# taraak/pita

Hardware: AMD Instinct MI355X
Metric: walker-steps/sec (batch x T) LJ13 @ 65k walkers/GPU (higher is better)
Workload: dtype f32

## Files before the change

pita_amd/csrc/egnn_div_kernel.hip:

```cpp
#include <type_traits>

#include "egnn_common.h"

namespace pita {

struct DivParams {
  const unsigned* mats16;
  const unsigned* mats16h;
  const float* vecs;
  const float* vecs_h;
  const float* vecs_div;
  float* cache;
  int* mark;
  int repair;
  int nchunk;
  int* bad_flag;
  int bad_seq;
  int n_layers, in_nf, attention, tanh_on, feature_layout;
  float coord_scale;
  long long B;
  const float* h;
  const float* x;
  const float* beta;
  int dir0, ndir;
  long long cache_waves;
  float* diag_acc;
  float* out;
  int no_mean;
  const float* probes;
  unsigned long long seed, walker_offset;
  long long step;
  float* q_out;
};

template <int N, int DIM>
__device__ __forceinline__ void probe_values(const DivParams& p, int probe, long long wid, int node, float (&v)[DIM]) {
  if (p.probes) {
    const float* src = p.probes + (((long long)probe * p.B + wid) * N + node) * DIM;
#pragma unroll
    for (int k = 0; k < DIM; ++k) v[k] = src[k];
  } else {
    const uint32_t word = philox_rademacher_word(p.seed, p.walker_offset + (unsigned long long)wid, p.step, (uint32_t)probe,
                                                 (uint32_t)node);
#pragma unroll
    for (int k = 0; k < DIM; ++k) v[k] = rademacher_sign(word, k);
  }
}

template <int N, int DIM, int POS_F>
__device__ __forceinline__ float probe_quadratic_form(const float* dscr, const float* vtab, int w, int d, float c_s, float cf) {
  const float* dF = dscr + d * POS_F + w * N * DIM;
  const float* vv = vtab + d * POS_F + w * N * DIM;
  float mean[DIM];
#pragma unroll
  for (int c = 0; c < DIM; ++c) {
    float s = 0.f;
    for (int j = 0; j < N; ++j) s += dF[j * DIM + c];
    mean[c] = s / (float)N;
  }
  float q = 0.f;
  for (int i = 0; i < N; ++i)
#pragma unroll
    for (int c = 0; c < DIM; ++c) {
      const float v = vv[i * DIM + c];
      q = fmaf(v, fmaf(cf, dF[i * DIM + c] - mean[c], c_s * v), q);
    }
  return q;
}

template <int N, int DIM, int G, int WAVES, int K, int DAL = 1>
struct DivCfg {
  static constexpr int NCOL = G * N;
  static constexpr int NT = (NCOL + 31) / 32;
  static constexpr int NCOLP = NT * 32;
  static constexpr int PB_F = NCOLP * PBS;
  static constexpr int POS_F = NCOLP * DIM;
  static constexpr int WAVE_F = (1 + K + DAL * K) * PB_F + 3 * POS_F + 3 * K * POS_F;
  static __host__ __device__ constexpr int vec_f(int L) { return ((VEC_EMB_F + L * VEC_LAYER_F) + 3) & ~3; }
  static __host__ __device__ constexpr size_t lds_bytes(int L) {
    return sizeof(float) * (size_t)(vec_f(L) + WAVES * WAVE_F + L * VEC_DIV_F);
  }
// ... 288 lines not shown
        }
      }
      wave_lds_fence();
      cur ^= 1;
    }

    float* dscr = dPB;
#pragma unroll
    for (int T = 0; T < NT; ++T)
#pragma unroll
      for (int d = 0; d < K; ++d)
#pragma unroll
        for (int k = 0; k < DIM; ++k) {
          dposi[T][d][k] -= dp0i[T][d][k];
          if (hh == 0) dscr[d * C::POS_F + col[T] * DIM + k] = dposi[T][d][k];
        }
    if constexpr (PROBE) {
      float* vtab = dA;
#pragma unroll
      for (int T = 0; T < NT; ++T) {
        const long long wid = valid[T] ? walker0 + col[T] / N : p.B - 1;
#pragma unroll
        for (int d = 0; d < K; ++d) {
          float pv[DIM];
          probe_values<N, DIM>(p, dir0 + (d < ndir ? d : 0), wid, nodei[T], pv);
          if (hh == 0) {
#pragma unroll
            for (int k = 0; k < DIM; ++k) vtab[d * C::POS_F + col[T] * DIM + k] = (valid[T] && d < ndir) ? pv[k] : 0.f;
          }
        }
      }
      wave_lds_fence();
      if (lane < G * K) {
        const int w = lane / K, d = lane - w * K;
        if (w < nwalk && d < ndir && (!p.repair || p.mark[walker0 + w] != 0)) {
          const float hv = p.h[walker0 + w];
          const float op = 1.0f + hv, rs = 1.0f / sqrtf(op);
          p.q_out[(long long)(dir0 + d) * p.B + walker0 + w] =
              probe_quadratic_form<N, DIM, C::POS_F>(dscr, vtab, w, d, 1.0f / op, sqrtf(hv) * rs);
        }
      }
      wave_lds_fence();
    } else {
    wave_lds_fence();
#pragma unroll
    for (int T = 0; T < NT; ++T) {
      const int cb = (col[T] < ncol) ? col[T] - nodei[T] : 0;
#pragma unroll
      for (int d = 0; d < K; ++d)
#pragma unroll
        for (int k = 0; k < DIM; ++k) {
          if (!(mine[T] && hh == 0 && d < ndir && nodei[T] * DIM + k == dir0 + d)) continue;
          float ds = 0.f;
          for (int q = 0; q < N; ++q) ds += dscr[d * C::POS_F + (cb + q) * DIM + k];
          const float dF = p.no_mean ? dposi[T][d][k] : dposi[T][d][k] - ds / (float)N;
          atomicAdd(&p.diag_acc[walker0 + col[T] / N], fmaf(c_out[T], dF, c_s[T]));
        }
    }
    wave_lds_fence();
    }
    if (p.out && ch == 0) {
      float* scr = PB;
#pragma unroll
      for (int T = 0; T < NT; ++T)
        if (hh == 0) {
#pragma unroll
          for (int k = 0; k < DIM; ++k) scr[col[T] * DIM + k] = posi[T][k] - p0i[T][k];
        }
      wave_lds_fence();
#pragma unroll
      for (int T = 0; T < NT; ++T) {
        if (!(mine[T] && hh == 0)) continue;
        const int cb = col[T] - nodei[T];
#pragma unroll
        for (int k = 0; k < DIM; ++k) {
          float sum = 0.f;
          for (int q = 0; q < N; ++q) sum += scr[(cb + q) * DIM + k];
          const float F = (posi[T][k] - p0i[T][k]) - sum / (float)N;
          const long long gi = (walker0 * N + col[T]) * DIM + k;
          p.out[gi] = fmaf(c_s[T], p.x[gi], c_out[T] * F);
        }
      }
      wave_lds_fence();
    }
    }
  }
}


template <int N, int DIM, int NT>
struct DivCache {
  static constexpr int POSX = NT * 32 * DIM;
  static constexpr int POSF = ((POSX + 2 * NT * 32 + 255) / 256) * 256;
  static __host__ __device__ int nvec(int l, int L) { return (l == 0 || l == L - 1) ? 1 : 4; }
  static __host__ __device__ size_t edge_f(int l, int L) { return (size_t)nvec(l, L) * 1024 + 512; }
  static __host__ __device__ size_t gn_off(int l, int L) { return (size_t)(N - 1) * edge_f(l, L); }
  static __host__ __device__ size_t tile_f(int l, int L) { return 1024 + (size_t)(N - 1) * edge_f(l, L); }
  static __host__ __device__ size_t layer_f(int l, int L) { return POSF + (size_t)NT * tile_f(l, L); }
  static __host__ __device__ size_t group_f(int L) {
    size_t t = 0;
    for (int l = 0; l < L; ++l) t += layer_f(l, L);
    return t;
  }
  static __host__ __device__ size_t layer_off(int l, int L) {
    size_t t = 0;
    for (int q = 0; q < l; ++q) t += layer_f(q, L);
    return t;
  }
// ... 408 lines not shown
          gn *= F16_UNSCALE;
          if (clay) cache_store16(clay + CA::POSF + (size_t)T * CA::tile_f(l, L) + CA::gn_off(l, L), lane, gn);
          wn.load(nullptr, mats16h, M_WN2, lane);
          f32x16 o = wn.mul(yn, lds_vec16(vl + V_BN2 * EH));
          o *= F16_UNSCALE;
          hf[T] += o;
#pragma unroll
          for (int d = 0; d < K; ++d) {
            dzn[d] *= gn;
            f32x16 dho = wn.mul(dzn[d], zero16);
            dho *= F16_UNSCALE;
            dhf[T][d] += dho;
          }
        }
      }
      wave_lds_fence();
      cur ^= 1;
    }

    float* dscr = dPB;
    float* tsl = PB;
#pragma unroll
    for (int T = 0; T < NT; ++T)
#pragma unroll
      for (int d = 0; d < K; ++d)
#pragma unroll
        for (int k = 0; k < DIM; ++k) {
          dposi[T][d][k] -= dp0i[T][d][k];
          if (hh == 0) dscr[d * C::POS_F + col[T] * DIM + k] = dposi[T][d][k];
        }
    if (lane < G * K) tsl[lane] = 0.f;
    if constexpr (PROBE) {
      const float* vtab = dpos0;
      wave_lds_fence();
      if (lane < G * K) {
        const int w = lane / KA, d = lane - w * KA;
        if (w < nwalk && d < p.ndir) {
          const float hv = p.h[walker0 + w];
          const float op = 1.0f + hv, rs = 1.0f / sqrtf(op);
          tsl[lane] = probe_quadratic_form<N, DIM, C::POS_F>(dscr, vtab, w, d, 1.0f / op, (sqrtf(hv) * rs) * rs);
        }
      }
    } else {
    wave_lds_fence();
#pragma unroll
    for (int T = 0; T < NT; ++T) {
      const int cb = (col[T] < ncol) ? col[T] - nodei[T] : 0;
#pragma unroll
      for (int d = 0; d < K; ++d)
#pragma unroll
        for (int k = 0; k < DIM; ++k) {
          if (!(valid[T] && hh == 0 && d < p.ndir && nodei[T] * DIM + k == p.dir0 + d)) continue;
          float ds = 0.f;
          for (int q = 0; q < N; ++q) ds += dscr[d * C::POS_F + (cb + q) * DIM + k];
          const float dF = p.no_mean ? dposi[T][d][k] : dposi[T][d][k] - ds / (float)N;
          tsl[(col[T] / N) * K + d] = fmaf(c_out[T] * c_in[T], dF, c_s[T]);
        }
    }
    }
    wave_lds_fence();
    bool bad[NT];
#pragma unroll
    for (int T = 0; T < NT; ++T) {
      bad[T] = false;
      if constexpr (K > 0) {
        const int w = col[T] / N;
        float sum = 0.f;
#pragma unroll
        for (int d = 0; d < K; ++d) sum += tsl[(valid[T] ? w : 0) * K + d];
        bad[T] = valid[T] && !__builtin_isfinite(sum);
        if (valid[T] && hh == 0 && nodei[T] == 0) {
          if constexpr (PROBE) {
            if (!bad[T])
#pragma unroll
              for (int d = 0; d < K; ++d)
                if (d < p.ndir) p.q_out[(long long)(p.dir0 + d) * p.B + walker0 + w] = tsl[w * K + d];
          } else {
            if (!bad[T]) p.diag_acc[walker0 + w] += sum;
          }
          p.mark[walker0 + w] = bad[T] ? 1 : 0;
          if (bad[T] && p.bad_flag) *p.bad_flag = p.bad_seq;
        }
      }
    }
    wave_lds_fence();
    if (p.out || K == 0) {
      float* scr = PB;
#pragma unroll
      for (int T = 0; T < NT; ++T)
        if (hh == 0) {
#pragma unroll
          for (int k = 0; k < DIM; ++k) scr[col[T] * DIM + k] = posi[T][k] - p0i[T][k];
        }
      wave_lds_fence();
#pragma unroll
      for (int T = 0; T < NT; ++T) {
        if (!(valid[T] && hh == 0) || bad[T]) continue;
        const int cb = col[T] - nodei[T];
        float F[DIM];
        bool fin = true;
#pragma unroll
        for (int k = 0; k < DIM; ++k) {
          float sum = 0.f;
          for (int q = 0; q < N; ++q) sum += scr[(cb + q) * DIM + k];
          F[k] = (posi[T][k] - p0i[T][k]) - sum / (float)N;
          fin = fin && __builtin_isfinite(F[k]);
        }
        if constexpr (K == 0) {
// ... 248 lines not shown
            if (hh == 0) dposb[(2 * d + (cur ^ 1)) * C::POS_F + col[T] * DIM + k] = dposi[T][d][k];
          }
        if (l != L - 1) {
          const f32x16 gn = cache_load16(ctile + CA::gn_off(l, L), lane);
          WFrag<2> wn;
          f32x16 dzn[K];
          if (!first) {
            wn.load(nullptr, mats16h, M_WN1A, lane);
#pragma unroll
            for (int d = 0; d < K; ++d) dzn[d] = wn.mul(dhf[T][d], zero16);
          } else {
#pragma unroll
            for (int d = 0; d < K; ++d) dzn[d] = zero16;
          }
          wn.load(nullptr, mats16h, M_WN1B, lane);
#pragma unroll
          for (int d = 0; d < K; ++d) dzn[d] = wn.mul(dagg[d], dzn[d]);
          wn.load(nullptr, mats16h, M_WN2, lane);
#pragma unroll
          for (int d = 0; d < K; ++d) {
            dzn[d] *= gn;
            f32x16 dho = wn.mul(dzn[d], zero16);
            dho *= F16_UNSCALE;
            dhf[T][d] += dho;
          }
        }
      }
      wave_lds_fence();
      cur ^= 1;
    }

    float* dscr = dPB;
    float* tsl = dPB + K * C::POS_F;
#pragma unroll
    for (int T = 0; T < NT; ++T)
#pragma unroll
      for (int d = 0; d < K; ++d)
#pragma unroll
        for (int k = 0; k < DIM; ++k) {
          dposi[T][d][k] -= dp0i[T][d][k];
          if (hh == 0) dscr[d * C::POS_F + col[T] * DIM + k] = dposi[T][d][k];
        }
    if (lane < G * K) tsl[lane] = 0.f;
    wave_lds_fence();
#pragma unroll
    for (int T = 0; T < NT; ++T) {
      const int cb = (col[T] < ncol) ? col[T] - nodei[T] : 0;
#pragma unroll
      for (int d = 0; d < K; ++d)
#pragma unroll
        for (int k = 0; k < DIM; ++k) {
          if (!(valid[T] && hh == 0 && d < p.ndir && nodei[T] * DIM + k == p.dir0 + d)) continue;
          float ds = 0.f;
          for (int q = 0; q < N; ++q) ds += dscr[d * C::POS_F + (cb + q) * DIM + k];
          const float dF = p.no_mean ? dposi[T][d][k] : dposi[T][d][k] - ds / (float)N;
          tsl[(col[T] / N) * K + d] = fmaf(cc[T], dF, c_s[T]);
        }
    }
    wave_lds_fence();
#pragma unroll
    for (int T = 0; T < NT; ++T) {
      const int w = col[T] / N;
      float sum = 0.f;
#pragma unroll
      for (int d = 0; d < K; ++d) sum += tsl[(valid[T] ? w : 0) * K + d];
      if (valid[T] && hh == 0 && nodei[T] == 0) {
        const bool bad = !__builtin_isfinite(sum);
        if (!bad) p.diag_acc[walker0 + w] += sum;
        p.mark[walker0 + w] = bad ? 1 : 0;
        if (bad && p.bad_flag) *p.bad_flag = p.bad_seq;
      }
    }
    wave_lds_fence();
  }
}


constexpr int SHR_LMAX = 4;
constexpr int SHR_S = 18;
template <int N, int DIM, int G, int NW, int K>
struct DivShrCfg {
  static constexpr int NCOL = G * N;
  static constexpr int NT = (NCOL + 31) / 32;
  static constexpr int NCOLP = NT * 32;
  static constexpr int PB_F = NCOLP * PBS;
  static constexpr int POS_F = NCOLP * DIM;
  static constexpr int WAVE_F = K * PB_F + 2 * K * POS_F;
  static constexpr int RES_G = 32;
  static constexpr bool COMPACT = NT * (N - 1) > 48;
  static constexpr int MAX_P = COMPACT ? 768 : 128 * NW;
  static constexpr int SHARED_F = 2 * POS_F + 2 * NCOLP + NW * G + RES_G * G + RES_G + MAX_P + 4;
  static constexpr int LMAX = SHR_LMAX;
  static __host__ __device__ constexpr int vec_f(int L) { return ((VEC_EMB_F + L * VEC_LAYER_F) + 3) & ~3; }
  static constexpr int FIXED_F = ((vec_f(LMAX) + SHARED_F + NW * WAVE_F) + 255) & ~255;
  static constexpr int NSLOT = (160 * 1024 - 4 * FIXED_F) / (SHR_S * 1024);
  static constexpr int D = (NW % 3 == 0 && NW / 3 >= NSLOT) ? 3 : ((NW % 2 == 0 && NW / 2 >= NSLOT) ? 2 : 1);
  static constexpr int PPW = SHR_S / D;
  static_assert(NSLOT >= 3 && NW / D >= NSLOT && SHR_S % D == 0, "ring / duty split");
  static __host__ __device__ constexpr size_t lds_bytes(int) { return (size_t)NSLOT * SHR_S * 1024 + sizeof(float) * (size_t)FIXED_F; }
};

__device__ __forceinline__ void lds_barrier() {
  asm volatile("s_waitcnt lgkmcnt(0)" ::: "memory");
  __builtin_amdgcn_s_barrier();
  asm volatile("" ::: "memory");
}
__device__ __forceinline__ void glds16s(unsigned lds_byte, const float* sbase, unsigned voff) {
  unsigned keep;
// ... 217 lines not shown
          p.mark[wid] = bad ? 1 : 0;
          if (bad && p.bad_flag) *p.bad_flag = p.bad_seq;
        }
      }
      asm volatile("s_waitcnt vmcnt(0)" ::: "memory");
    }
    nres = 0;
  };

  for (int gid = next_group(blockIdx.x); gid < ngroups_i; gid = next_group(gid + nblk)) {
    long long walker0;
    const int nwalk = group_walkers(gid, walker0);
    const int ncol = nwalk * N;
    const int ntile = (ncol + 31) >> 5;
    int col[NT], nodei[NT];
    bool valid[NT];
    float dposi[NT][K][DIM];
    auto unit = [&](int T, int q, int k) -> float {
      return (valid[T] && q < myndir && nodei[T] * DIM + k == mydir0 + q) ? 1.0f : 0.f;
    };
    f32x16 dhf[NT][K];
    int dnode[K], dk[K];
    float si[NT][K];
#pragma unroll
    for (int q = 0; q < K; ++q) {
      const int dq = mydir0 + q;
      dnode[q] = (q < myndir) ? dq / DIM : -1;
      dk[q] = dq - (dq / DIM) * DIM;
    }
#pragma unroll
    for (int T = 0; T < NT; ++T) {
      col[T] = T * 32 + cl;
      const int w = col[T] / N;
      nodei[T] = col[T] - w * N;
      valid[T] = col[T] < ncol;
#pragma unroll
      for (int q = 0; q < K; ++q) si[T][q] = (valid[T] && nodei[T] == dnode[q]) ? 2.0f : 0.0f;
#pragma unroll
      for (int k = 0; k < DIM; ++k)
#pragma unroll
        for (int q = 0; q < K; ++q) {
          const float v = unit(T, q, k);
          dposi[T][q][k] = v;
          if (hh == 0) {
            dposb[(2 * q) * C::POS_F + col[T] * DIM + k] = v;
            dposb[(2 * q + 1) * C::POS_F + col[T] * DIM + k] = 0.f;
          }
        }
#pragma unroll
      for (int q = 0; q < K; ++q) dhf[T][q] = zero16;
    }

    constexpr int EPI2 = S / 6;
    static_assert(G * K * EPI2 <= 32, "virtual columns of the last layer");
    auto vcol = [&](int& v_e, int& v_d, int& v_w, int& v_i0, int& v_k0, bool& v_on, int& v_col0, int& v_c0) {
      v_e = cl % EPI2; v_d = (cl / EPI2) % K; v_w = cl / (EPI2 * K);
      v_i0 = 0; v_k0 = 0;
#pragma unroll
      for (int q = 0; q < K; ++q) {
        v_i0 = (v_d == q) ? dnode[q] : v_i0;
        v_k0 = (v_d == q) ? dk[q] : v_k0;
      }
      v_on = active && v_w < nwalk && v_w < G && v_i0 >= 0;
      v_col0 = v_on ? v_w * N + v_i0 : 0;
      v_c0 = v_col0 & 31;
    };
    float vacc[DIM];
#pragma unroll
    for (int k = 0; k < DIM; ++k) vacc[k] = 0.f;

    int cur = 0;
    auto layer = [&](const int l, auto kind_tag) {
      constexpr bool first = decltype(kind_tag)::value == 0;
      constexpr bool last = decltype(kind_tag)::value == 2;
      const int nwm = first ? 0 : (last ? 2 : 3);
      begin_item();
      {
        const float* ipos = item + nwm * MAT_WH;
        if (first)
          for (int i = threadIdx.x; i < 2 * C::NCOLP; i += NW * 64) cstab[i] = ipos[CA::POSX + i];
      }
      WFrag<2> w2f;
      f32x16 dArT[NT][K];
      if (!first && active) {
        {
          const WFrag<2> wa = slot_wfrag(item, 0, lane);
#pragma unroll
          for (int T = 0; T < NT; ++T) {
            if (T >= ntile) continue;
#pragma unroll
            for (int d = 0; d < K; ++d) {
              dArT[T][d] = wa.mul(dhf[T][d], zero16);
              dArT[T][d] *= F16_UNSCALE;
            }
          }
        }
        const WFrag<2> wb = slot_wfrag(item, 1, lane);
        if (!last) w2f = slot_wfrag(item, 2, lane);
#pragma unroll
        for (int T = 0; T < NT; ++T) {
          if (T >= ntile) continue;
#pragma unroll
          for (int d = 0; d < K; ++d) {
            f32x16 dpb = wb.mul(dhf[T][d], zero16);
            dpb *= F16_UNSCALE;
            f32x4* ddst = reinterpret_cast<f32x4*>(dPB + d * C::PB_F + col[T] * PBS + hh * 16);
#pragma unroll
            for (int q = 0; q < 4; ++q) ddst[q] = f32x4{dpb[4 * q], dpb[4 * q + 1], dpb[4 * q + 2], dpb[4 * q + 3]};
          }
        }
      }
      end_item();
      const float a_re = vecs[VEC_EMB_F + l * VEC_LAYER_F + V_WRE * EH + lane];
      const float aggw = (l == L - 1) ? 0.0f : 1.0f;
#pragma unroll
      for (int T = 0; T < NT; ++T) {
// ... 220 lines not shown
              f32x4* dst = reinterpret_cast<f32x4*>(aggT + ca * PBS);
#pragma unroll
              for (int q = 0; q < 4; ++q) dst[q] = f32x4{v[4 * q], v[4 * q + 1], v[4 * q + 2], v[4 * q + 3]};
              if (hh == 0) {
#pragma unroll
                for (int k = 0; k < DIM; ++k) posT[ca * DIM + k] = x[k];
              }
            }
            if (on && !f_s) {
              accA += v;
#pragma unroll
              for (int k = 0; k < DIM; ++k) accX[k] += x[k];
            }
            end_item();
          }
          {
#pragma unroll
            for (int r = 0; r < 16; ++r) {
              float t = accA[r];
#pragma unroll
              for (int e = 1; e < EPI2; ++e) t += __shfl_down(accA[r], e, 64);
              accA[r] = t;
            }
#pragma unroll
            for (int k = 0; k < DIM; ++k) {
              float t = accX[k];
#pragma unroll
              for (int e = 1; e < EPI2; ++e) t += __shfl_down(accX[k], e, 64);
              accX[k] = t;
            }
            const int c0g = f_w * N + f_i0;
            if (f_on && !f_s && f_e == 0 && (c0g >> 5) == T) {
              f32x4* dst = reinterpret_cast<f32x4*>(aggT + c0g * PBS);
#pragma unroll
              for (int q = 0; q < 4; ++q) dst[q] = f32x4{accA[4 * q], accA[4 * q + 1], accA[4 * q + 2], accA[4 * q + 3]};
              if (hh == 0) {
#pragma unroll
                for (int k = 0; k < DIM; ++k) posT[c0g * DIM + k] = ((f_k0 == k) ? 1.0f : 0.0f) + accX[k];
              }
            }
          }
          wave_lds_fence();
          if (tile_on) {
#pragma unroll
            for (int d = 0; d < K; ++d) {
              const bool has = valid[T] && d < myndir;
              dagg[d] = has ? lds_vec16(dPB + d * C::PB_F + col[T] * PBS + hh * 16) : zero16;
#pragma unroll
              for (int k = 0; k < DIM; ++k)
                dposi[T][d][k] = has ? dposb[(2 * d + (cur ^ 1)) * C::POS_F + col[T] * DIM + k] : 0.0f;
            }
          }
        } else if (last) {
          int v_e, v_d, v_w, v_i0, v_k0, v_col0, v_c0;
          bool v_on;
          vcol(v_e, v_d, v_w, v_i0, v_k0, v_on, v_col0, v_c0);
          const bool mine = v_on && (v_col0 >> 5) == T && tile_on;
          f32x16 dAv = zero16;
#pragma unroll
          for (int q = 0; q < K; ++q)
#pragma unroll
            for (int r = 0; r < 16; ++r) {
              const float t = __shfl(dAr[q][r], v_c0 + 32 * hh, 64);
              dAv[r] = (v_d == q) ? t : dAv[r];
            }
          const float* vdpos = dposb + (2 * v_d + cur) * C::POS_F;
          const float* vdPB = dPB + v_d * C::PB_F + hh * 16;
#pragma unroll 1
          for (int dd0 = 1; dd0 < N; dd0 += EPI2) {
            begin_item();
            const int dd = dd0 + v_e;
            const bool on = mine && dd < N;
            int j = v_i0 + (on ? dd : 0);
            j = (j >= N) ? j - N : j;
            const int cj = on ? v_w * N + j : 0;
            const float* rec = item + v_e * (1024 + 512);
            const float* sc = rec + 1024;
            const float cs = sc[v_c0], dcs_f = sc[64 + v_c0], qr = sc[256 + v_c0], qe = sc[320 + v_c0];
            const f32x4 ga = *reinterpret_cast<const f32x4*>(sc + 128 + v_c0 * 4);
            const f32x4 gb = *reinterpret_cast<const f32x4*>(sc + 384 + v_c0 * 4);
            float df[DIM], e0[DIM];
            df[0] = ga.x; e0[0] = gb.x;
            df[1] = ga.y; e0[1] = gb.y;
            if constexpr (DIM > 2) { df[DIM - 1] = ga.z; e0[DIM - 1] = gb.z; }
            const float inv = ga.w, hsq = gb.w;
            float ddf[DIM], dradial = 0.f, e0k = e0[0];
#pragma unroll
            for (int k = 0; k < DIM; ++k) {
              ddf[k] = vdpos[v_col0 * DIM + k] - vdpos[cj * DIM + k];
              dradial = fmaf(df[k], ddf[k], dradial);
              if (k > 0) e0k = (v_k0 == k) ? e0[k] : e0k;
            }
            dradial *= 2.0f;
            const float dea = 2.0f * e0k;
            f32x16 qv;
            {
              const f32x4* qp = reinterpret_cast<const f32x4*>(rec) + (hh * 32 + v_c0);
#pragma unroll
              for (int q = 0; q < 4; ++q) {
                const f32x4 t = qp[q * 64];
                qv[4 * q] = t.x; qv[4 * q + 1] = t.y; qv[4 * q + 2] = t.z; qv[4 * q + 3] = t.w;
              }
            }
            const f32x16 dz1 = dAv + lds_vec16(vdPB + cj * PBS);
            const float sdot = xhalf_sum(dot16(qv, dz1));
            const float dcs = dcs_f * fmaf(qr, dradial, fmaf(qe, dea, sdot));
            const float dnrm = dradial * hsq;
#pragma unroll
            for (int k = 0; k < DIM; ++k) {
              const float u = df[k] * inv;
              const float du = (ddf[k] - u * dnrm) * inv;
              const float t = fmaf(du, cs, u * dcs);
              vacc[k] += on ? t : 0.0f;
            }
            end_item();
          }
        } else if (first) run_edges(std::integral_constant<int, 0>{});
        else run_edges(std::integral_constant<int, 1>{});
        if (tile_on && !last && !(first && VFIRST)) {
#pragma unroll
          for (int k = 0; k < DIM; ++k)
#pragma unroll
            for (int d = 0; d < K; ++d) {
              dposi[T][d][k] += dxacc[d][k];
              if (hh == 0) dposb[(2 * d + (cur ^ 1)) * C::POS_F + col[T] * DIM + k] = dposi[T][d][k];
            }
        }
        const int nnm = (l == L - 1) ? 0 : (first ? 2 : 3);
        begin_item();
        if (tile_on && l != L - 1) {
          const f32x16 gn = slot_vec16(item, nnm, lane);
          f32x16 dzn[K];
          if (!first) {
            const WFrag<2> wn = slot_wfrag(item, 0, lane);
#pragma unroll
            for (int d = 0; d < K; ++d) dzn[d] = wn.mul(dhf[T][d], zero16);
          } else {
#pragma unroll
            for (int d = 0; d < K; ++d) dzn[d] = zero16;
          }
          {
            const WFrag<2> wn = slot_wfrag(item, nnm - 2, lane);
#pragma unroll
            for (int d = 0; d < K; ++d) dzn[d] = wn.mul(dagg[d], dzn[d]);
          }
          const WFrag<2> wn = slot_wfrag(item, nnm - 1, lane);
#pragma unroll
          for (int d = 0; d < K; ++d) {
            dzn[d] *= gn;
            f32x16 dho = wn.mul(dzn[d], zero16);
            dho *= F16_UNSCALE;
            dhf[T][d] += dho;
          }
        }
        end_item();
      }
      cur ^= 1;
    };
    layer(0, std::integral_constant<int, 0>{});
    for (int l = 1; l < L - 1; ++l) layer(l, std::integral_constant<int, 1>{});
    layer(L - 1, std::integral_constant<int, 2>{});

    float* tsl = dPB + K * C::POS_F;
    wave_lds_fence();
    {
      int v_e, v_d, v_w, v_i0, v_k0, v_col0, v_c0;
      bool v_on;
      vcol(v_e, v_d, v_w, v_i0, v_k0, v_on, v_col0, v_c0);
      float tot[DIM];
#pragma unroll
      for (int k = 0; k < DIM; ++k) {
        tot[k] = vacc[k];
#pragma unroll
        for (int e = 1; e < EPI2; ++e) tot[k] += __shfl_down(vacc[k], e, 64);
      }
      if (lane < G * K) tsl[lane] = 0.f;
      wave_lds_fence();
      if (v_on && hh == 0 && v_e == 0) {
        const float* vdpos = dposb + (2 * v_d + (cur ^ 1)) * C::POS_F;
        float tk = tot[0], pk = vdpos[v_col0 * DIM];
#pragma unroll
        for (int k = 1; k < DIM; ++k) {
          tk = (v_k0 == k) ? tot[k] : tk;
          pk = (v_k0 == k) ? vdpos[v_col0 * DIM + k] : pk;
        }
        const float dF = (pk + tk) - 1.0f;
        tsl[v_w * K + v_d] = fmaf(cstab[C::NCOLP + v_col0], dF, cstab[v_col0]);
      }
    }
    wave_lds_fence();
    if (lane < G) {
      float sum = 0.f;
#pragma unroll
      for (int d = 0; d < K; ++d) sum += tsl[lane * K + d];
      comb[wave * G + lane] = sum;
    }
    lds_barrier();
    if (wave == 0 && lane < G) {
      float sum = 0.f;
      for (int w = 0; w < NW; ++w) sum += comb[w * G + lane];
      res[nres * G + lane] = (lane < nwalk) ? sum : -0.0f;
      if (lane == 0) resw[nres] = (int)walker0;
    }
    ++nres;
    if (nres == C::RES_G) {
      wave_lds_fence();
      flush();
    }
  }
  wave_lds_fence();
  flush();
}

struct DivKernel {
  void (*kernel)(DivParams) = nullptr;
  size_t (*lds_bytes)(int) = nullptr;
  int waves = 0, K = 0;
  bool (*fits)(int) = nullptr;
};
struct DivSystem {
  int n, dim, G, waves, K;
  DivKernel bf16x3;
  DivKernel f16;
  DivKernel writer;
  DivKernel shared, owned;
  size_t (*group_f)(int);
  DivKernel bf16x3_probe, f16_probe;
};
template <int N, int DIM, int G, int WAVES, int K, int DAL>
static size_t div_lds_bytes_of(int L) { return DivCfg<N, DIM, G, WAVES, K, DAL>::lds_bytes(L); }
template <int N, int DIM, int G, int WAVES, int K>
static size_t divtan_lds_of(int L) { return DivTanCfg<N, DIM, G, WAVES, K>::lds_bytes(L); }
template <int N, int DIM, int G, int NW, int K>
static size_t divshr_lds_of(int L) { return DivShrCfg<N, DIM, G, NW, K>::lds_bytes(L); }
template <int N, int DIM, int G>
static size_t divcache_group_f(int L) { return DivCache<N, DIM, (G * N + 31) / 32>::group_f(L); }
template <int N, int DIM, int G, int NW, int K>
static bool divshr_fits(int L) {
  using C = DivShrCfg<N, DIM, G, NW, K>;
  using CA = DivCache<N, DIM, C::NT>;
  if (L > SHR_LMAX || L < 2) return false;
  long long items = 0;
  for (int l = 0; l < L; ++l) {
    const int epi = SHR_S / (int)(CA::edge_f(l, L) / 256);
    items += 1 + (long long)C::NT * ((N - 1 + epi - 1) / epi + 1);
  }
  return items * (C::COMPACT ? 2 : SHR_S) <= C::MAX_P;
}
template <int N, int DIM, int G, int WAVES, int K, bool WRITER, int SHR_NW, int SHR_K, int OWN_K>
static DivSystem div_system() {
  DivSystem s{N, DIM, G, WAVES, K,
              {egnn_div_kernel<N, DIM, G, WAVES, K>, div_lds_bytes_of<N, DIM, G, WAVES, K, 1>, WAVES, K},
              {egnn_div_fast_kernel<N, DIM, G, WAVES, K, 1>, div_lds_bytes_of<N, DIM, G, WAVES, K, 1>, WAVES, K},
              {}, {}, {}, divcache_group_f<N, DIM, G>};
  s.bf16x3_probe = {egnn_div_kernel<N, DIM, G, WAVES, K, DivProbes>, div_lds_bytes_of<N, DIM, G, WAVES, K, 1>, WAVES, K};
  s.f16_probe = {egnn_div_fast_kernel<N, DIM, G, WAVES, K, 1, 1, DivProbes>, div_lds_bytes_of<N, DIM, G, WAVES, K, 1>, WAVES, K};
  if constexpr (WRITER)
    s.writer = {egnn_div_fast_kernel<N, DIM, G, WAVES, 0, 0, 1>, div_lds_bytes_of<N, DIM, G, WAVES, 0, 0>, WAVES, 0};
  if constexpr (SHR_K > 0)
    s.shared = {egnn_div_tangent_shared_kernel<N, DIM, G, SHR_NW, SHR_K>, divshr_lds_of<N, DIM, G, SHR_NW, SHR_K>, SHR_NW,
                SHR_K, divshr_fits<N, DIM, G, SHR_NW, SHR_K>};
  if constexpr (OWN_K > 0)
    s.owned = {egnn_div_tangent_kernel<N, DIM, G, WAVES, OWN_K>, divtan_lds_of<N, DIM, G, WAVES, OWN_K>, WAVES, OWN_K};
  return s;
}
static const DivSystem kDivSystems[] = {
    div_system<4,  2,  8, 4,    3, false, 0,     0,     5>(),
    div_system<13, 3,  2, 4,    3, true,  8,     2,     4>(),
    div_system<22, 3,  1, 4,    3, true,  8,     2,     4>(),
    div_system<55, 3,  1, 4,    1, false, 8,     1,     3>(),
};

struct DivPlan {
  const DivSystem* sys = nullptr;
  bool f16 = false;
  const DivKernel* first = nullptr;
  const DivKernel* tangent = nullptr;
};
static DivPlan div_plan(const pita_egnn* net) {
  DivPlan pl;
  for (const auto& s : kDivSystems)
    if (s.n == net->cfg.n_particles && s.dim == net->cfg.n_dim) pl.sys = &s;
  if (!pl.sys) return pl;
  const DivSystem& s = *pl.sys;
  pl.f16 = net->cfg.precision == 2;
  if (!pl.f16 || s.n * s.dim <= s.K) return pl;
  if (s.shared.kernel && s.shared.fits(net->cfg.n_layers)) {
    pl.tangent = &s.shared;
    pl.first = s.writer.kernel ? &s.writer : &s.f16;
  } else if (s.owned.kernel) {
    pl.tangent = &s.owned;
    pl.first = &s.f16;
  }
  return pl;
}

struct DivGrid {
  long long grid, waves, groups_per_wave;
};
static DivGrid div_grid(const pita_egnn* net, const DivSystem& s, long long B) {
  const long long ngroups = (B + s.G - 1) / s.G;
  const long long want = (ngroups + s.waves - 1) / s.waves;
  const long long grid = want < net->n_cu ? want : net->n_cu;
  const long long waves = grid * s.waves;
  const long long quota = (B + waves - 1) / waves;
  return {grid, waves, (quota + s.G - 1) / s.G};
}

static DivParams div_params(const pita_egnn* net) {
  DivParams p{};
  p.mats16 = net->d_mats16; p.mats16h = net->d_mats16h; p.vecs = net->d_vecs; p.vecs_h = net->d_vecs_h;
  p.vecs_div = net->d_vecs_div;
  p.n_layers = net->cfg.n_layers; p.in_nf = net->cfg.in_node_nf;
  p.attention = net->cfg.attention; p.tanh_on = net->cfg.tanh; p.feature_layout = net->cfg.feature_layout;
  p.coord_scale = net->cfg.coords_range / (float)net->cfg.n_layers;
  return p;
}

static int div_launch(const DivKernel& k, long long grid, const DivParams& p, hipStream_t st) {
  const size_t lds = k.lds_bytes(p.n_layers);
  PITA_HIP_CHECK(ensure_dynamic_lds(reinterpret_cast<const void*>(k.kernel), lds));
// ... 21 lines not shown
}

using namespace pita;

extern "C" int pita_egnn_div_directions(const pita_egnn_t* net) {
  if (!net) return PITA_EINVAL;
  const DivPlan pl = div_plan(net);
  return pl.sys ? pl.sys->K : PITA_EUNSUPPORTED;
}

extern "C" int pita_egnn_div_work(const pita_egnn_t* net, double* mfma16_per_walker, double* mfma32_per_walker) {
  PITA_REQUIRE(net && mfma16_per_walker && mfma32_per_walker, "pita_egnn_div_work: null argument");
  const DivPlan pl = div_plan(net);
  if (!pl.sys) return fail(PITA_EUNSUPPORTED, "pita_egnn_div_work: no kernel for this particle system");
  const DivSystem& s = *pl.sys;
  const int N = s.n, L = net->cfg.n_layers, D = s.n * s.dim;
  const int K = pl.first ? pl.first->K : s.K;
  const double tiles_per_walker = (double)((s.G * N + 31) / 32) / s.G;
  double m16 = 0, m32 = 0, t16 = 0, t32 = 0;
  if (pl.f16) {
    for (int l = 0; l < L; ++l) {
      const bool first = l == 0, lastl = l == L - 1;
      m16 += 12 + (N - 1) * 18.0 + (lastl ? 0 : 18);
      m32 += N - 1;
      if (first) m16 += (N - 1) * 6.0;
      else if (lastl) m16 += (N - 1) * 6.0;
      else { m16 += (N - 1) * 6.0 * K; m32 += (N - 1) * K; }
      if (!first) m16 += 12.0 * K + (lastl ? 0 : 6.0 * K);
      if (!lastl) m16 += 12.0 * K;
      if (!first) t16 += 12.0 + (lastl ? 0 : 6.0);
      if (!first && !lastl) { t16 += (N - 1) * 6.0; t32 += N - 1; }
      if (!lastl) t16 += 12.0;
    }
  } else {
    for (int l = 0; l < L; ++l) {
      const bool first = l == 0, lastl = l == L - 1;
      m16 += 24 + (N - 1) * 24.0 + (lastl ? 0 : 36);
      m32 += N - 1;
      m16 += K * ((N - 1) * 24.0 + (first ? 0 : 24) + (lastl ? 0 : (first ? 24 : 36)));
      m32 += K * (N - 1);
    }
  }
  if (pl.first) {
    *mfma16_per_walker = (m16 + (D - K) * t16) * tiles_per_walker;
    *mfma32_per_walker = (m32 + (D - K) * t32) * tiles_per_walker;
    return PITA_OK;
  }
  const double launches = (D + K - 1) / K;
  *mfma16_per_walker = m16 * tiles_per_walker * launches;
  *mfma32_per_walker = m32 * tiles_per_walker * launches;
  return PITA_OK;
}

extern "C" int pita_egnn_div_accumulate(pita_egnn_t* net, const float* h, const float* x, const float* beta, int dir0,
                                        int ndir, float* diag_acc, float* out, int64_t B, void* stream) {
  PITA_REQUIRE(net && B >= 0, "pita_egnn_div_accumulate: bad argument");
  if (B == 0) return PITA_OK;
  PitaDeviceGuard guard(net->device);
  PITA_REQUIRE(h && x && diag_acc, "pita_egnn_div_accumulate: null argument");
  PITA_REQUIRE(beta || net->cfg.in_node_nf == 1, "pita_egnn_div_accumulate: beta required for in_node_nf=2");
  const DivPlan pl = div_plan(net);
  if (!pl.sys) return fail(PITA_EUNSUPPORTED, "pita_egnn_div_accumulate: no kernel for this particle system");
  const DivSystem& s = *pl.sys;
  PITA_REQUIRE(dir0 >= 0 && ndir >= 1 && ndir <= s.K && dir0 + ndir <= s.n * s.dim,
               "pita_egnn_div_accumulate: directions out of range");
  hipStream_t st = (hipStream_t)stream;
  DivParams p = div_params(net);
  p.B = B; p.h = h; p.x = x; p.beta = beta; p.dir0 = dir0; p.ndir = ndir; p.diag_acc = diag_acc; p.out = out;
  const long long grid = div_grid(net, s, B).grid;
  if (!pl.f16) return div_launch(s.bf16x3, grid, p, st);
  const int rc = ensure_marks(net, (size_t)B, st);
  if (rc != PITA_OK) return rc;
  p.mark = net->d_mark;
  p.bad_flag = net->d_mark + net->mark_bytes / sizeof(int);
  p.bad_seq = ++net->div_seq;
  const int rc1 = div_launch(s.f16, grid, p, st);
  if (rc1 != PITA_OK) return rc1;
  p.repair = 1;
  return div_launch(s.bf16x3, grid, p, st);
}

static int div_trace_uncached(pita_egnn_t* net, int K, const float* h, const float* x, const float* beta, float* trace,
                              float* denoiser_out, int64_t B, void* stream) {
  const int D = net->cfg.n_particles * net->cfg.n_dim;
  for (int d0 = 0; d0 < D; d0 += K) {
    const int rc = pita_egnn_div_accumulate(net, h, x, beta, d0, (D - d0) < K ? (D - d0) : K, trace,
                                            d0 == 0 ? denoiser_out : nullptr, B, stream);
    if (rc != PITA_OK) return rc;
  }
  return PITA_OK;
}

extern "C" int pita_egnn_jacobian_trace(pita_egnn_t* net, const float* h, const float* x, const float* beta, float* trace,
                                        float* denoiser_out, int64_t B, void* stream) {
  PITA_REQUIRE(net && B >= 0, "pita_egnn_jacobian_trace: bad argument");
  if (B == 0) return PITA_OK;
  PitaDeviceGuard guard(net->device);
  PITA_REQUIRE(h && x && trace, "pita_egnn_jacobian_trace: null argument");
  PITA_REQUIRE(beta || net->cfg.in_node_nf == 1, "pita_egnn_jacobian_trace: beta required for in_node_nf=2");
  const DivPlan pl = div_plan(net);
  if (!pl.sys) return fail(PITA_EUNSUPPORTED, "pita_egnn_jacobian_trace: no kernel for this particle system");
  const DivSystem& s = *pl.sys;
  const int D = s.n * s.dim, L = net->cfg.n_layers;
  hipStream_t st = (hipStream_t)stream;
  PITA_HIP_CHECK(hipMemsetAsync(trace, 0, sizeof(float) * (size_t)B, st));
  if (!pl.tangent) return div_trace_uncached(net, s.K, h, x, beta, trace, denoiser_out, B, stream);
  double budget_gb = 24.0;
  if (getenv("PITA_DIV_CACHE_GB")) {
    budget_gb = atof(getenv("PITA_DIV_CACHE_GB"));
  } else {
    size_t free_b = 0, total_b = 0;
    if (hipMemGetInfo(&free_b, &total_b) == hipSuccess) {
      const double avail = 0.6 * ((double)free_b + (double)net->divcache_bytes) / 1e9;
      if (avail < budget_gb) budget_gb = avail;
    } else {
      (void)hipGetLastError();
    }
  }
  const double per_walker = 4.0 * (double)s.group_f(L) / s.G;
  long long chunk = (long long)(budget_gb * 1e9 / per_walker);
  chunk = chunk / 1024 * 1024;
  if (chunk < 1024) chunk = 1024;
  if (chunk > B) chunk = B;
  auto cache_need = [&](long long Bc) -> size_t {
    const DivGrid g = div_grid(net, s, Bc);
    return sizeof(float) * s.group_f(L) * (size_t)(g.waves * g.groups_per_wave);
  };
  while (grow_scratch(net->d_divcache, net->divcache_bytes, cache_need(chunk), st) != hipSuccess) {
    (void)hipGetLastError();
    if (chunk <= 1024) return div_trace_uncached(net, s.K, h, x, beta, trace, denoiser_out, B, stream);
    chunk = (chunk / 2 + 1023) / 1024 * 1024;
  }
  const DivKernel& tk = *pl.tangent;
  const bool shared = pl.tangent == &s.shared;
  const int per_launch = shared ? tk.K * tk.waves : tk.K;
  for (long long b0 = 0; b0 < B; b0 += chunk) {
    const long long Bc = (B - b0) < chunk ? (B - b0) : chunk;
    const DivGrid g = div_grid(net, s, Bc);
    PITA_REQUIRE(cache_need(Bc) <= net->divcache_bytes, "pita_egnn_jacobian_trace: cache smaller than a chunk");
    PITA_REQUIRE(g.waves * g.groups_per_wave < 0x7fffffffLL && Bc < 0x7fffffffLL,
                 "pita_egnn_jacobian_trace: too many walkers in one chunk");
    const int rc0 = ensure_marks(net, (size_t)Bc, st);
    if (rc0 != PITA_OK) return rc0;
    DivParams p = div_params(net);
    p.B = Bc; p.h = h + b0; p.x = x + b0 * D; p.beta = beta ? beta + b0 : nullptr; p.diag_acc = trace + b0;
    p.no_mean = 1;
    p.mark = net->d_mark;
    p.bad_flag = net->d_mark + net->mark_bytes / sizeof(int);
    p.cache = net->d_divcache;
    p.cache_waves = g.waves;
    auto repair = [&](int dir0, int ndir, float* out) -> int {
      DivParams r = p;
      r.repair = 1;
      r.cache = nullptr;
      if (ndir == 0) {
        if (!out) return PITA_OK;
        r.dir0 = 0; r.ndir = 0; r.out = out;
        return div_launch(s.bf16x3, g.grid, r, st);
      }
      r.dir0 = dir0;
      r.ndir = ndir;
      r.nchunk = (ndir + s.K - 1) / s.K;
      r.out = out;
      return div_launch(s.bf16x3, g.grid, r, st);
    };
    p.dir0 = 0; p.ndir = pl.first->K < D ? pl.first->K : D; p.out = denoiser_out ? denoiser_out + b0 * D : nullptr;
    p.bad_seq = ++net->div_seq;
    int rc = div_launch(*pl.first, g.grid, p, st);
    if (rc != PITA_OK) return rc;
    rc = repair(0, p.ndir, p.out);
    if (rc != PITA_OK) return rc;
    p.out = nullptr;
    const long long groups = g.waves * g.groups_per_wave;
    const long long tgrid = !shared ? g.grid : (groups < (long long)net->n_cu ? groups : (long long)net->n_cu);
    for (int d0 = pl.first->K; d0 < D; d0 += per_launch) {
      p.dir0 = d0;
      p.ndir = (D - d0) < per_launch ? (D - d0) : per_launch;
      p.bad_seq = ++net->div_seq;
      rc = div_launch(tk, tgrid, p, st);
      if (rc != PITA_OK) return rc;
      rc = repair(d0, p.ndir, nullptr);
      if (rc != PITA_OK) return rc;
    }
  }
  return PITA_OK;
}

extern "C" int pita_egnn_trace_probes(pita_egnn_t* net, const float* h, const float* x, const float* beta, int n_probes,
                                      const float* probes, uint64_t seed, uint64_t walker_offset, int64_t step,
                                      float* estimate, float* per_probe, float* denoiser_out, int64_t B, void* stream) {
  PITA_REQUIRE(net && B >= 0, "pita_egnn_trace_probes: bad argument");
  PITA_REQUIRE(n_probes >= 1, "pita_egnn_trace_probes: n_probes must be at least 1");
  PITA_REQUIRE(probes || n_probes <= kMaxDrawnProbes, "pita_egnn_trace_probes: probes drawn in the kernel need n_probes <= %d",
               kMaxDrawnProbes);
  if (B == 0) return PITA_OK;
  PITA_REQUIRE(h && x && estimate, "pita_egnn_trace_probes: null argument");
  PITA_REQUIRE(beta || net->cfg.in_node_nf == 1, "pita_egnn_trace_probes: beta required for in_node_nf=2");
  const DivPlan pl = div_plan(net);
  if (!pl.sys) return fail(PITA_EUNSUPPORTED, "pita_egnn_trace_probes: no kernel for this particle system");
  const DivSystem& s = *pl.sys;
  PITA_REQUIRE((long long)n_probes * B < (1LL << 40), "pita_egnn_trace_probes: too many (probe, walker) pairs");
  PitaDeviceGuard guard(net->device);
  hipStream_t st = (hipStream_t)stream;
  float* q = per_probe;
  if (!q) {
    PITA_HIP_CHECK(grow_scratch(net->d_probe_q, net->probe_q_bytes, sizeof(float) * (size_t)n_probes * (size_t)B, st));
    q = net->d_probe_q;
  }
  DivParams p = div_params(net);
  p.B = B; p.h = h; p.x = x; p.beta = beta; p.q_out = q;
  p.probes = probes; p.seed = seed; p.walker_offset = walker_offset; p.step = step;
  if (pl.f16) {
    const int rc = ensure_marks(net, (size_t)B, st);
    if (rc != PITA_OK) return rc;
    p.mark = net->d_mark;
    p.bad_flag = net->d_mark + net->mark_bytes / sizeof(int);
  }
  const long long grid = div_grid(net, s, B).grid;
  for (int k0 = 0; k0 < n_probes; k0 += s.K) {
    p.dir0 = k0;
    p.ndir = (n_probes - k0) < s.K ? (n_probes - k0) : s.K;
    p.out = k0 == 0 ? denoiser_out : nullptr;
    p.repair = 0;
    int rc;
    if (!pl.f16) {
      rc = div_launch(s.bf16x3_probe, grid, p, st);
    } else {
      p.bad_seq = ++net->div_seq;
      rc = div_launch(s.f16_probe, grid, p, st);
      if (rc != PITA_OK) return rc;
      p.repair = 1;
      rc = div_launch(s.bf16x3_probe, grid, p, st);
// ... 9 lines not shown
```

Measured before the change: 63.36 million.

## Fold last particle's directions into trace via translation invariance, add K=1 tail kernel

Uses translation invariance of the EGNN to skip the last particle's Jacobian directions. The trace is initialised with dim/(1+h), and the other directions subtract the last node's response (fold_last), so D-dim directions are evaluated instead of N*dim. In the shared tangent kernel the last layer doubles its virtual columns to compute the last-node term and combines the two with a shuffle. A K=1 shared kernel instantiation handles a small final direction batch for LJ13. The result relies on the model being exactly translation-equivariant, and the doubled virtual columns add work to each last-layer pass.

```diff
diff --git a/pita_amd/csrc/egnn_div_kernel.hip b/pita_amd/csrc/egnn_div_kernel.hip
--- a/pita_amd/csrc/egnn_div_kernel.hip
+++ b/pita_amd/csrc/egnn_div_kernel.hip
@@ -27,6 +27,7 @@
   float* diag_acc;
   float* out;
   int no_mean;
+  int fold_last;
   const float* probes;
   unsigned long long seed, walker_offset;
   long long step;
@@ -421,8 +422,10 @@
         for (int k = 0; k < DIM; ++k) {
           if (!(mine[T] && hh == 0 && d < ndir && nodei[T] * DIM + k == dir0 + d)) continue;
           float ds = 0.f;
-          for (int q = 0; q < N; ++q) ds += dscr[d * C::POS_F + (cb + q) * DIM + k];
-          const float dF = p.no_mean ? dposi[T][d][k] : dposi[T][d][k] - ds / (float)N;
+          if (!p.fold_last)
+            for (int q = 0; q < N; ++q) ds += dscr[d * C::POS_F + (cb + q) * DIM + k];
+          const float dF = p.fold_last ? dposi[T][d][k] - dscr[d * C::POS_F + (cb + N - 1) * DIM + k]
+                                       : (p.no_mean ? dposi[T][d][k] : dposi[T][d][k] - ds / (float)N);
           atomicAdd(&p.diag_acc[walker0 + col[T] / N], fmaf(c_out[T], dF, c_s[T]));
         }
     }
@@ -937,8 +940,10 @@
         for (int k = 0; k < DIM; ++k) {
           if (!(valid[T] && hh == 0 && d < p.ndir && nodei[T] * DIM + k == p.dir0 + d)) continue;
           float ds = 0.f;
-          for (int q = 0; q < N; ++q) ds += dscr[d * C::POS_F + (cb + q) * DIM + k];
-          const float dF = p.no_mean ? dposi[T][d][k] : dposi[T][d][k] - ds / (float)N;
+          if (!p.fold_last)
+            for (int q = 0; q < N; ++q) ds += dscr[d * C::POS_F + (cb + q) * DIM + k];
+          const float dF = p.fold_last ? dposi[T][d][k] - dscr[d * C::POS_F + (cb + N - 1) * DIM + k]
+                                       : (p.no_mean ? dposi[T][d][k] : dposi[T][d][k] - ds / (float)N);
           tsl[(col[T] / N) * K + d] = fmaf(c_out[T] * c_in[T], dF, c_s[T]);
         }
     }
@@ -1293,8 +1298,10 @@
         for (int k = 0; k < DIM; ++k) {
           if (!(valid[T] && hh == 0 && d < p.ndir && nodei[T] * DIM + k == p.dir0 + d)) continue;
           float ds = 0.f;
-          for (int q = 0; q < N; ++q) ds += dscr[d * C::POS_F + (cb + q) * DIM + k];
-          const float dF = p.no_mean ? dposi[T][d][k] : dposi[T][d][k] - ds / (float)N;
+          if (!p.fold_last)
+            for (int q = 0; q < N; ++q) ds += dscr[d * C::POS_F + (cb + q) * DIM + k];
+          const float dF = p.fold_last ? dposi[T][d][k] - dscr[d * C::POS_F + (cb + N - 1) * DIM + k]
+                                       : (p.no_mean ? dposi[T][d][k] : dposi[T][d][k] - ds / (float)N);
           tsl[(col[T] / N) * K + d] = fmaf(cc[T], dF, c_s[T]);
         }
     }
@@ -1618,16 +1625,18 @@
     }
 
     constexpr int EPI2 = S / 6;
-    static_assert(G * K * EPI2 <= 32, "virtual columns of the last layer");
-    auto vcol = [&](int& v_e, int& v_d, int& v_w, int& v_i0, int& v_k0, bool& v_on, int& v_col0, int& v_c0) {
-      v_e = cl % EPI2; v_d = (cl / EPI2) % K; v_w = cl / (EPI2 * K);
-      v_i0 = 0; v_k0 = 0;
+    static_assert(G * K * 2 * EPI2 <= 32, "virtual columns of the last layer");
+    auto vcol = [&](int& v_e, int& v_s, int& v_d, int& v_w, int& v_dn, int& v_i0, int& v_k0, bool& v_on, int& v_col0,
+                    int& v_c0) {
+      v_e = cl % EPI2; v_s = (cl / EPI2) & 1; v_d = (cl / (2 * EPI2)) % K; v_w = cl / (2 * EPI2 * K);
+      v_dn = 0; v_k0 = 0;
 #pragma unroll
       for (int q = 0; q < K; ++q) {
-        v_i0 = (v_d == q) ? dnode[q] : v_i0;
+        v_dn = (v_d == q) ? dnode[q] : v_dn;
         v_k0 = (v_d == q) ? dk[q] : v_k0;
       }
-      v_on = active && v_w < nwalk && v_w < G && v_i0 >= 0;
+      v_i0 = v_s ? N - 1 : v_dn;
+      v_on = active && v_w < nwalk && v_w < G && v_dn >= 0;
       v_col0 = v_on ? v_w * N + v_i0 : 0;
       v_c0 = v_col0 & 31;
     };
@@ -1954,9 +1963,9 @@
             }
           }
         } else if (last) {
-          int v_e, v_d, v_w, v_i0, v_k0, v_col0, v_c0;
+          int v_e, v_s, v_d, v_w, v_dn, v_i0, v_k0, v_col0, v_c0;
           bool v_on;
-          vcol(v_e, v_d, v_w, v_i0, v_k0, v_on, v_col0, v_c0);
+          vcol(v_e, v_s, v_d, v_w, v_dn, v_i0, v_k0, v_on, v_col0, v_c0);
           const bool mine = v_on && (v_col0 >> 5) == T && tile_on;
           f32x16 dAv = zero16;
 #pragma unroll
@@ -1994,7 +2003,7 @@
               if (k > 0) e0k = (v_k0 == k) ? e0[k] : e0k;
             }
             dradial *= 2.0f;
-            const float dea = 2.0f * e0k;
+            const float dea = v_s ? ((j == v_dn) ? -2.0f * e0k : 0.0f) : 2.0f * e0k;
             f32x16 qv;
             {
               const f32x4* qp = reinterpret_cast<const f32x4*>(rec) + (hh * 32 + v_c0);
@@ -2066,9 +2075,9 @@
     float* tsl = dPB + K * C::POS_F;
     wave_lds_fence();
     {
-      int v_e, v_d, v_w, v_i0, v_k0, v_col0, v_c0;
+      int v_e, v_s, v_d, v_w, v_dn, v_i0, v_k0, v_col0, v_c0;
       bool v_on;
-      vcol(v_e, v_d, v_w, v_i0, v_k0, v_on, v_col0, v_c0);
+      vcol(v_e, v_s, v_d, v_w, v_dn, v_i0, v_k0, v_on, v_col0, v_c0);
       float tot[DIM];
 #pragma unroll
       for (int k = 0; k < DIM; ++k) {
@@ -2078,17 +2087,17 @@
       }
       if (lane < G * K) tsl[lane] = 0.f;
       wave_lds_fence();
-      if (v_on && hh == 0 && v_e == 0) {
-        const float* vdpos = dposb + (2 * v_d + (cur ^ 1)) * C::POS_F;
-        float tk = tot[0], pk = vdpos[v_col0 * DIM];
-#pragma unroll
-        for (int k = 1; k < DIM; ++k) {
-          tk = (v_k0 == k) ? tot[k] : tk;
-          pk = (v_k0 == k) ? vdpos[v_col0 * DIM + k] : pk;
-        }
-        const float dF = (pk + tk) - 1.0f;
-        tsl[v_w * K + v_d] = fmaf(cstab[C::NCOLP + v_col0], dF, cstab[v_col0]);
-      }
+      const float* vdpos = dposb + (2 * v_d + (cur ^ 1)) * C::POS_F;
+      float tk = tot[0], pk = vdpos[v_col0 * DIM];
+#pragma unroll
+      for (int k = 1; k < DIM; ++k) {
+        tk = (v_k0 == k) ? tot[k] : tk;
+        pk = (v_k0 == k) ? vdpos[v_col0 * DIM + k] : pk;
+      }
+      const float dFs = v_s ? pk + tk : (pk + tk) - 1.0f;
+      const float dFlast = __shfl_down(dFs, EPI2, 64);
+      if (v_on && hh == 0 && v_e == 0 && v_s == 0)
+        tsl[v_w * K + v_d] = fmaf(cstab[C::NCOLP + v_col0], dFs - dFlast, cstab[v_col0]);
     }
     wave_lds_fence();
     if (lane < G) {
@@ -2128,6 +2137,7 @@
   DivKernel shared, owned;
   size_t (*group_f)(int);
   DivKernel bf16x3_probe, f16_probe;
+  DivKernel shared1;
 };
 template <int N, int DIM, int G, int WAVES, int K, int DAL>
 static size_t div_lds_bytes_of(int L) { return DivCfg<N, DIM, G, WAVES, K, DAL>::lds_bytes(L); }
@@ -2149,7 +2159,7 @@
   }
   return items * (C::COMPACT ? 2 : SHR_S) <= C::MAX_P;
 }
-template <int N, int DIM, int G, int WAVES, int K, bool WRITER, int SHR_NW, int SHR_K, int OWN_K>
+template <int N, int DIM, int G, int WAVES, int K, bool WRITER, int SHR_NW, int SHR_K, int OWN_K, bool SHR_TAIL1 = false>
 static DivSystem div_system() {
   DivSystem s{N, DIM, G, WAVES, K,
               {egnn_div_kernel<N, DIM, G, WAVES, K>, div_lds_bytes_of<N, DIM, G, WAVES, K, 1>, WAVES, K},
@@ -2162,13 +2172,16 @@
   if constexpr (SHR_K > 0)
     s.shared = {egnn_div_tangent_shared_kernel<N, DIM, G, SHR_NW, SHR_K>, divshr_lds_of<N, DIM, G, SHR_NW, SHR_K>, SHR_NW,
                 SHR_K, divshr_fits<N, DIM, G, SHR_NW, SHR_K>};
+  if constexpr (SHR_TAIL1)
+    s.shared1 = {egnn_div_tangent_shared_kernel<N, DIM, G, SHR_NW, 1>, divshr_lds_of<N, DIM, G, SHR_NW, 1>, SHR_NW, 1,
+                 divshr_fits<N, DIM, G, SHR_NW, 1>};
   if constexpr (OWN_K > 0)
     s.owned = {egnn_div_tangent_kernel<N, DIM, G, WAVES, OWN_K>, divtan_lds_of<N, DIM, G, WAVES, OWN_K>, WAVES, OWN_K};
   return s;
 }
 static const DivSystem kDivSystems[] = {
     div_system<4,  2,  8, 4,    3, false, 0,     0,     5>(),
-    div_system<13, 3,  2, 4,    3, true,  8,     2,     4>(),
+    div_system<13, 3,  2, 4,    3, true,  8,     2,     4,       true>(),
     div_system<22, 3,  1, 4,    3, true,  8,     2,     4>(),
     div_system<55, 3,  1, 4,    1, false, 8,     1,     3>(),
 };
@@ -2296,8 +2309,8 @@
   return PITA_OK;
 }
 
-extern "C" int pita_egnn_div_accumulate(pita_egnn_t* net, const float* h, const float* x, const float* beta, int dir0,
-                                        int ndir, float* diag_acc, float* out, int64_t B, void* stream) {
+static int div_accumulate(pita_egnn_t* net, const float* h, const float* x, const float* beta, int dir0, int ndir,
+                          float* diag_acc, float* out, int64_t B, void* stream, int fold) {
   PITA_REQUIRE(net && B >= 0, "pita_egnn_div_accumulate: bad argument");
   if (B == 0) return PITA_OK;
   PitaDeviceGuard guard(net->device);
@@ -2311,6 +2324,7 @@
   hipStream_t st = (hipStream_t)stream;
   DivParams p = div_params(net);
   p.B = B; p.h = h; p.x = x; p.beta = beta; p.dir0 = dir0; p.ndir = ndir; p.diag_acc = diag_acc; p.out = out;
+  p.fold_last = fold;
   const long long grid = div_grid(net, s, B).grid;
   if (!pl.f16) return div_launch(s.bf16x3, grid, p, st);
   const int rc = ensure_marks(net, (size_t)B, st);
@@ -2324,15 +2338,39 @@
   return div_launch(s.bf16x3, grid, p, st);
 }
 
+extern "C" int pita_egnn_div_accumulate(pita_egnn_t* net, const float* h, const float* x, const float* beta, int dir0,
+                                        int ndir, float* diag_acc, float* out, int64_t B, void* stream) {
+  return div_accumulate(net, h, x, beta, dir0, ndir, diag_acc, out, B, stream, 0);
+}
+
 static int div_trace_uncached(pita_egnn_t* net, int K, const float* h, const float* x, const float* beta, float* trace,
                               float* denoiser_out, int64_t B, void* stream) {
-  const int D = net->cfg.n_particles * net->cfg.n_dim;
+  const int D = (net->cfg.n_particles - 1) * net->cfg.n_dim;
   for (int d0 = 0; d0 < D; d0 += K) {
-    const int rc = pita_egnn_div_accumulate(net, h, x, beta, d0, (D - d0) < K ? (D - d0) : K, trace,
-                                            d0 == 0 ? denoiser_out : nullptr, B, stream);
+    const int rc = div_accumulate(net, h, x, beta, d0, (D - d0) < K ? (D - d0) : K, trace,
+                                  d0 == 0 ? denoiser_out : nullptr, B, stream, 1);
     if (rc != PITA_OK) return rc;
   }
   return PITA_OK;
+}
+
+__global__ void __launch_bounds__(256) egnn_trace_init_kernel(const float* __restrict__ h, float* __restrict__ trace,
+                                                              long long B, float dim) {
+  const long long b = (long long)blockIdx.x * blockDim.x + threadIdx.x;
+  if (b >= B) return;
+  trace[b] = dim * (1.0f / (1.0f + h[b]));
+}
+
+struct DivTracePlan {
+  int full, tail_k1;
+};
+static DivTracePlan div_trace_plan(const DivSystem& s) {
+  DivTracePlan tp{s.shared.K * s.shared.waves, 1};
+  if (const char* e = getenv("PITA_DIV_TRACE_PLAN")) {
+    int full = 0, k1 = 0;
+    if (sscanf(e, "%d,%d", &full, &k1) == 2 && full >= 1 && full <= tp.full) tp = {full, k1 != 0};
+  }
+  return tp;
 }
 
 extern "C" int pita_egnn_jacobian_trace(pita_egnn_t* net, const float* h, const float* x, const float* beta, float* trace,
@@ -2345,9 +2383,11 @@
   const DivPlan pl = div_plan(net);
   if (!pl.sys) return fail(PITA_EUNSUPPORTED, "pita_egnn_jacobian_trace: no kernel for this particle system");
   const DivSystem& s = *pl.sys;
-  const int D = s.n * s.dim, L = net->cfg.n_layers;
+  const int D = s.n * s.dim, DF = (s.n - 1) * s.dim, L = net->cfg.n_layers;
   hipStream_t st = (hipStream_t)stream;
-  PITA_HIP_CHECK(hipMemsetAsync(trace, 0, sizeof(float) * (size_t)B, st));
+  hipLaunchKernelGGL(egnn_trace_init_kernel, dim3((unsigned)((B + 255) / 256)), dim3(256), 0, st, h, trace, (long long)B,
+                     (float)s.dim);
+  PITA_LAUNCH_CHECK();
   if (!pl.tangent) return div_trace_uncached(net, s.K, h, x, beta, trace, denoiser_out, B, stream);
   double budget_gb = 24.0;
   if (getenv("PITA_DIV_CACHE_GB")) {
@@ -2377,7 +2417,9 @@
   }
   const DivKernel& tk = *pl.tangent;
   const bool shared = pl.tangent == &s.shared;
-  const int per_launch = shared ? tk.K * tk.waves : tk.K;
+  const DivTracePlan tp = shared ? div_trace_plan(s) : DivTracePlan{tk.K, 0};
+  const int per_launch = tp.full;
+  const bool tail1 = tp.tail_k1 && s.shared1.kernel && s.shared1.fits(L);
   for (long long b0 = 0; b0 < B; b0 += chunk) {
     const long long Bc = (B - b0) < chunk ? (B - b0) : chunk;
     const DivGrid g = div_grid(net, s, Bc);
@@ -2389,6 +2431,7 @@
     DivParams p = div_params(net);
     p.B = Bc; p.h = h + b0; p.x = x + b0 * D; p.beta = beta ? beta + b0 : nullptr; p.diag_acc = trace + b0;
     p.no_mean = 1;
+    p.fold_last = 1;
     p.mark = net->d_mark;
     p.bad_flag = net->d_mark + net->mark_bytes / sizeof(int);
     p.cache = net->d_divcache;
@@ -2408,7 +2451,7 @@
       r.out = out;
       return div_launch(s.bf16x3, g.grid, r, st);
     };
-    p.dir0 = 0; p.ndir = pl.first->K < D ? pl.first->K : D; p.out = denoiser_out ? denoiser_out + b0 * D : nullptr;
+    p.dir0 = 0; p.ndir = pl.first->K < DF ? pl.first->K : DF; p.out = denoiser_out ? denoiser_out + b0 * D : nullptr;
     p.bad_seq = ++net->div_seq;
     int rc = div_launch(*pl.first, g.grid, p, st);
     if (rc != PITA_OK) return rc;
@@ -2417,11 +2460,12 @@
     p.out = nullptr;
     const long long groups = g.waves * g.groups_per_wave;
     const long long tgrid = !shared ? g.grid : (groups < (long long)net->n_cu ? groups : (long long)net->n_cu);
-    for (int d0 = pl.first->K; d0 < D; d0 += per_launch) {
+    for (int d0 = pl.first->K; d0 < DF; d0 += per_launch) {
       p.dir0 = d0;
-      p.ndir = (D - d0) < per_launch ? (D - d0) : per_launch;
+      p.ndir = (DF - d0) < per_launch ? (DF - d0) : per_launch;
       p.bad_seq = ++net->div_seq;
-      rc = div_launch(tk, tgrid, p, st);
+      const bool k1 = tail1 && d0 + per_launch >= DF && p.ndir <= s.shared1.waves;
+      rc = div_launch(k1 ? s.shared1 : tk, tgrid, p, st);
       if (rc != PITA_OK) return rc;
       rc = repair(d0, p.ndir, nullptr);
       if (rc != PITA_OK) return rc;
```

New measurement: 63.35 million, median of 2. No clear change (-0.0%).
